# rqhuang88/DV-Matcher

Measured on AMD Instinct MI355X. Metric: point-cloud pairs/sec (N=2048, d=128), higher is better.
Workload: dtype f32; 1 GPU; BASELINE configs[1]: synthetic random pairs N=M=2048 d=128, correspondence+deform forward, both directions; deformer_weights=reference ckpt/dvmatcher_scape_r (fixture), fps_start=0, parallelism=pairs sharded over 1 GPU(s), no collective

## Files before the change

### dv-matcher_amd/csrc/dvm_grid.hip

```cpp
#include <stdlib.h>

#include <type_traits>

#include "dvm_common.h"

namespace dvm {

constexpr int GRID_T = 256;

template <class IndexT>
struct GridViewT {
    const float4 *pts;
    const IndexT *ids;
    const IndexT *start;
    float ox, oy, oz, h, scale2;
    int G;
};
typedef GridViewT<int32_t> GridView;
typedef GridViewT<uint16_t> GridViewLds;


static int grid_dim_for(int P) {
    int g = 2;
    while (g < 16 && (double)(g + 1) * (g + 1) * (g + 1) * 1.2 <= (double)P * 1.15) ++g;
    return g < 4 ? 4 : g;
}

struct GridBuildSets {
    const float *xyz[4];
    int Nsrc[4];
    GridBuf gb[4];
};
template <bool SETS>
__device__ __forceinline__ void grid_build_body(const float *__restrict__ xyz, int Nsrc, const int32_t *__restrict__ sel, const GridBuf &gb);
__global__ __launch_bounds__(GRID_T) void grid_build_sets_kernel(const GridBuildSets sets) {
    const int q = blockIdx.y;
    grid_build_body<true>(sets.xyz[q], sets.Nsrc[q], nullptr, sets.gb[q]);
}
__global__ __launch_bounds__(GRID_T) void grid_build_kernel(const float *__restrict__ xyz, int Nsrc,
                                                            const int32_t *__restrict__ sel, GridBuf gb) {
    grid_build_body<false>(xyz, Nsrc, sel, gb);
}
template <bool SETS>
__device__ __forceinline__ void grid_build_body(const float *__restrict__ xyz, int Nsrc, const int32_t *__restrict__ sel, const GridBuf &gb) {
    extern __shared__ int lds[];
    __shared__ float red[6][GRID_T / 64];
    __shared__ float par[8];
    __shared__ int wsum[GRID_T / 64];
    const int b = blockIdx.x, tid = threadIdx.x, lane = tid & 63, wave = tid >> 6;
    const int P = gb.P, G = gb.G, G3 = G * G * G;
    const float *p = xyz + (size_t)b * Nsrc * 3;
    const int32_t *sl = sel ? sel + (size_t)b * P : nullptr;
    constexpr int GC = 8;
    const bool cached = P <= GC * GRID_T;
    float px[GC], py[GC], pz[GC];
    if (cached) {
        int vs[GC];
#pragma unroll
        for (int q = 0; q < GC; ++q) {
            const int j = tid + q * GRID_T, jc = j < P ? j : P - 1;
            vs[q] = sl ? sl[jc] : jc;
        }
#pragma unroll
        for (int q = 0; q < GC; ++q) px[q] = p[3 * vs[q]], py[q] = p[3 * vs[q] + 1], pz[q] = p[3 * vs[q] + 2];
    }
    auto each_point = [&](auto &&f) __attribute__((always_inline)) {
        if (cached) {
#pragma unroll
            for (int q = 0; q < GC; ++q) {
                const int j = tid + q * GRID_T;
                if (j < P) f(j, px[q], py[q], pz[q]);
            }
        } else {
            for (int j = tid; j < P; j += GRID_T) {
                const int v = sl ? sl[j] : j;
                f(j, p[3 * v], p[3 * v + 1], p[3 * v + 2]);
            }
        }
    };
    float mn[3] = {INFINITY, INFINITY, INFINITY}, mx[3] = {-INFINITY, -INFINITY, -INFINITY};
    each_point([&](int, float x, float y, float z) {
        mn[0] = fminf(mn[0], x), mn[1] = fminf(mn[1], y), mn[2] = fminf(mn[2], z);
        mx[0] = fmaxf(mx[0], x), mx[1] = fmaxf(mx[1], y), mx[2] = fmaxf(mx[2], z);
    });
    for (int a = 0; a < 3; ++a) {
        for (int o = 32; o > 0; o >>= 1) {
            mn[a] = fminf(mn[a], __shfl_xor(mn[a], o, 64));
            mx[a] = fmaxf(mx[a], __shfl_xor(mx[a], o, 64));
        }
        if (lane == 0) {
            red[a][wave] = mn[a];
            red[3 + a][wave] = mx[a];
        }
    }
    __syncthreads();
    if (tid == 0) {
        float lo[3], hi[3];
        for (int a = 0; a < 3; ++a) {
            lo[a] = fminf(fminf(red[a][0], red[a][1]), fminf(red[a][2], red[a][3]));
            hi[a] = fmaxf(fmaxf(red[3 + a][0], red[3 + a][1]), fmaxf(red[3 + a][2], red[3 + a][3]));
        }
        float ext = fmaxf(fmaxf(hi[0] - lo[0], hi[1] - lo[1]), hi[2] - lo[2]);
        float h = ext > 0.f ? (ext / (float)G) * 1.000001f : 1.f;
        float m = 0.f;
        for (int a = 0; a < 3; ++a) m = fmaxf(m, fmaxf(fabsf(lo[a]), fabsf(hi[a])));
        par[0] = lo[0], par[1] = lo[1], par[2] = lo[2], par[3] = h, par[4] = 3.f * m * m + 1e-30f;
        for (int q = 0; q < 5; ++q) gb.params[(size_t)b * 8 + q] = par[q];
    }
    for (int c = tid; c <= G3; c += GRID_T) lds[c] = 0;
    __syncthreads();
    const float ox = par[0], oy = par[1], oz = par[2], inv = 1.0f / par[3];
    auto cell_of = [&](float x, float y, float z) {
        int cx = (int)((x - ox) * inv), cy = (int)((y - oy) * inv), cz = (int)((z - oz) * inv);
        cx = cx < 0 ? 0 : (cx > G - 1 ? G - 1 : cx);
        cy = cy < 0 ? 0 : (cy > G - 1 ? G - 1 : cy);
        cz = cz < 0 ? 0 : (cz > G - 1 ? G - 1 : cz);
        return (cz * G + cy) * G + cx;
    };
    each_point([&](int, float x, float y, float z) { atomicAdd(&lds[cell_of(x, y, z)], 1); });
    __syncthreads();
    const int chunk = (G3 + GRID_T - 1) / GRID_T;
    int local = 0;
    for (int c = tid * chunk; c < (tid + 1) * chunk && c < G3; ++c) local += lds[c];
    int inc = local;
    for (int o = 1; o < 64; o <<= 1) {
        int t = __shfl_up(inc, o, 64);
        if (lane >= o) inc += t;
    }
    if (lane == 63) wsum[wave] = inc;
    __syncthreads();
    int base = inc - local;
    for (int w2 = 0; w2 < wave; ++w2) base += wsum[w2];
    __syncthreads();
    int *cursor = lds + G3 + 1;
    int run = base;
    for (int c = tid * chunk; c < (tid + 1) * chunk && c < G3; ++c) {
        int cnt = lds[c];
        lds[c] = run;
        cursor[c] = run;
        run += cnt;
    }
    if (tid == 0) lds[G3] = P;
    __syncthreads();
    int32_t *st = gb.start + (size_t)b * (G3 + 1);
    for (int c = tid; c <= G3; c += GRID_T) st[c] = lds[c];
    float4 *op = gb.pts + (size_t)b * P;
    int32_t *oi = gb.ids + (size_t)b * P;
    each_point([&](int j, float x, float y, float z) {
        const int pos = atomicAdd(&cursor[cell_of(x, y, z)], 1);
        op[pos] = make_float4(x, y, z, sumsq3(x, y, z));
        oi[pos] = j;
    });
}

__device__ __forceinline__ GridView grid_view(const GridBuf &gb, int b) {
    GridView g;
    const int G3 = gb.G * gb.G * gb.G;
    g.pts = gb.pts + (size_t)b * gb.P;
    g.ids = gb.ids + (size_t)b * gb.P;
    g.start = gb.start + (size_t)b * (G3 + 1);
    const float *pr = gb.params + (size_t)b * 8;
    g.ox = pr[0], g.oy = pr[1], g.oz = pr[2], g.h = pr[3], g.scale2 = pr[4];
    g.G = gb.G;
    return g;
}

struct MetricMMQueryRow {
    typedef float key_t;
    float qx, qy, qz, nq;
    __device__ __forceinline__ void set(float x, float y, float z) { qx = x, qy = y, qz = z, nq = sumsq3(x, y, z); }
    __device__ __forceinline__ float operator()(const float4 &c) const {
        return sqrt_rn(d2_mm3(qx, qy, qz, nq, c.x, c.y, c.z, c.w));
    }
    __device__ __forceinline__ static float to_d2(float k) { return k * k; }
};
struct MetricMMCandRow {
    typedef float key_t;
    float qx, qy, qz, nq;
    __device__ __forceinline__ void set(float x, float y, float z) { qx = x, qy = y, qz = z, nq = sumsq3(x, y, z); }
    __device__ __forceinline__ float operator()(const float4 &c) const {
        return sqrt_rn(d2_mm3(c.x, c.y, c.z, c.w, qx, qy, qz, nq));
    }
    __device__ __forceinline__ static float to_d2(float k) { return k * k; }
};
struct MetricF64 {
    typedef double key_t;
    float qx, qy, qz;
    __device__ __forceinline__ void set(float x, float y, float z) { qx = x, qy = y, qz = z; }
    __device__ __forceinline__ double operator()(const float4 &c) const {
        double dx = (double)qx - (double)c.x, dy = (double)qy - (double)c.y, dz = (double)qz - (double)c.z;
        double s = 0.0;
        s = s + dx * dx;
        s = s + dy * dy;
        s = s + dz * dz;
        return s;
    }
    __device__ __forceinline__ static float to_d2(double k) { return (float)k; }
};
struct MetricF64Rounded {
    typedef float key_t;
    MetricF64 m;
    __device__ __forceinline__ void set(float x, float y, float z) { m.set(x, y, z); }
    __device__ __forceinline__ float operator()(const float4 &c) const { return (float)m(c); }
    __device__ __forceinline__ static float to_d2(float k) { return k; }
};
struct MetricDiff {
    typedef float key_t;
    float qx, qy, qz;
    __device__ __forceinline__ void set(float x, float y, float z) { qx = x, qy = y, qz = z; }
    __device__ __forceinline__ float operator()(const float4 &c) const { return d2_diff3(qx, qy, qz, c.x, c.y, c.z); }
    __device__ __forceinline__ static float to_d2(float k) { return k; }
};

template <class View, class Metric, class List>
__device__ __forceinline__ void grid_row(const View &g, const Metric &met, List &kb, int s0, int s1) {
    for (int s = s0; s < s1; ++s) kb.insert_lex(met(g.pts[s]), (int)g.ids[s]);
}

struct ChamferMin {
    float key;
    __device__ __forceinline__ float worst() const { return key; }
};
template <class Metric>
__device__ __forceinline__ void grid_row(const GridView &g, const Metric &met, ChamferMin &kb, int s0, int s1) {
    for (; s0 < s1; s0 += 4) {
        float4 pc[4];
#pragma unroll
        for (int u = 0; u < 4; ++u) pc[u] = g.pts[s0 + u < s1 ? s0 + u : s1 - 1];
#pragma unroll
        for (int u = 0; u < 4; ++u) kb.key = fminf(kb.key, s0 + u < s1 ? met(pc[u]) : INFINITY);
    }
}
struct ChamferMinPos {
    float key;
    int pos;
    __device__ __forceinline__ float worst() const { return key; }
};
template <class Metric>
__device__ __forceinline__ void grid_row(const GridView &g, const Metric &met, ChamferMinPos &kb, int s0, int s1) {
    for (int s = s0; s < s1; ++s) {
        const float v = met(g.pts[s]);
        if (v < kb.key) {
            kb.key = v, kb.pos = s;
        } else if (v == kb.key && (kb.pos < 0 || g.ids[s] < g.ids[kb.pos])) {
            kb.pos = s;
        }
    }
}

template <int K, class Metric, class List, class View>
__device__ __forceinline__ bool grid_search(const View &g, float qx, float qy, float qz, Metric &met, List &kb,
                                            int R0 = 1 , int Rmax = 1 << 30) {
    const int G = g.G;
    const float inv = 1.0f / g.h;
    int cx = (int)((qx - g.ox) * inv), cy = (int)((qy - g.oy) * inv), cz = (int)((qz - g.oz) * inv);
    cx = cx < 0 ? 0 : (cx > G - 1 ? G - 1 : cx);
    cy = cy < 0 ? 0 : (cy > G - 1 ? G - 1 : cy);
    cz = cz < 0 ? 0 : (cz > G - 1 ? G - 1 : cz);
    const float q2 = sumsq3(qx, qy, qz);
    const float margin = 64.f * 1.1920929e-7f * (g.scale2 + q2) + 1e-30f;
    int Rprev = R0 > 1 ? R0 - 1 : -1;
    for (int R = R0; R <= G && R <= Rmax; ++R) {
        const int x0 = cx - R < 0 ? 0 : cx - R, x1 = cx + R > G - 1 ? G - 1 : cx + R;
        const int y0 = cy - R < 0 ? 0 : cy - R, y1 = cy + R > G - 1 ? G - 1 : cy + R;
        const int z0 = cz - R < 0 ? 0 : cz - R, z1 = cz + R > G - 1 ? G - 1 : cz + R;
        for (int z = z0; z <= z1; ++z) {
            const float zlo = g.oz + (float)z * g.h;
            const float dz = fmaxf(0.f, fmaxf(zlo - qz, qz - (zlo + g.h)));
            for (int y = y0; y <= y1; ++y) {
                const float ylo = g.oy + (float)y * g.h;
                const float dy = fmaxf(0.f, fmaxf(ylo - qy, qy - (ylo + g.h)));
                if (Metric::to_d2(kb.worst()) < (dy * dy + dz * dz) * 0.9999f - margin) continue;
                const int rowbase = (z * G + y) * G;
                const bool inner_zy = (abs(z - cz) <= Rprev) && (abs(y - cy) <= Rprev);
                int sa0, sa1, sb0 = 0, sb1 = 0;
                if (inner_zy) {
                    const int ix0 = cx - Rprev < 0 ? 0 : cx - Rprev;
                    const int ix1 = cx + Rprev > G - 1 ? G - 1 : cx + Rprev;
                    sa0 = g.start[rowbase + x0];
                    sa1 = g.start[rowbase + ix0];
                    sb0 = g.start[rowbase + ix1 + 1];
                    sb1 = g.start[rowbase + x1 + 1];
                } else {
                    sa0 = g.start[rowbase + x0];
                    sa1 = g.start[rowbase + x1 + 1];
                }
                grid_row(g, met, kb, sa0, sa1);
                grid_row(g, met, kb, sb0, sb1);
            }
        }
        const float ext = (float)G * g.h;
        const float ex = fmaxf(0.f, fmaxf(g.ox - qx, qx - (g.ox + ext)));
        const float ey = fmaxf(0.f, fmaxf(g.oy - qy, qy - (g.oy + ext)));
        const float ez = fmaxf(0.f, fmaxf(g.oz - qz, qz - (g.oz + ext)));
        const float exx = ex * ex, eyy = ey * ey, ezz = ez * ez;
        float bound2 = INFINITY;
        auto face_x = [&](float f) { f = fmaxf(f, 0.f); bound2 = fminf(bound2, f * f + eyy + ezz); };
        auto face_y = [&](float f) { f = fmaxf(f, 0.f); bound2 = fminf(bound2, f * f + exx + ezz); };
        auto face_z = [&](float f) { f = fmaxf(f, 0.f); bound2 = fminf(bound2, f * f + exx + eyy); };
        if (cx - R >= 1) face_x(qx - (g.ox + (float)(cx - R) * g.h));
        if (cx + R < G - 1) face_x((g.ox + (float)(cx + R + 1) * g.h) - qx);
        if (cy - R >= 1) face_y(qy - (g.oy + (float)(cy - R) * g.h));
        if (cy + R < G - 1) face_y((g.oy + (float)(cy + R + 1) * g.h) - qy);
        if (cz - R >= 1) face_z(qz - (g.oz + (float)(cz - R) * g.h));
        if (cz + R < G - 1) face_z((g.oz + (float)(cz + R + 1) * g.h) - qz);
        if (bound2 == INFINITY) return true;
        const float kth = Metric::to_d2(kb.worst());
        if (kth < bound2 * 0.9999f - margin) return true;
        Rprev = R;
    }
    return Rmax >= G;
}

static __host__ __device__ __forceinline__ size_t grid_lds_bytes(int P, int G) {
    return ((size_t)P * (sizeof(float4) + sizeof(uint16_t)) + ((size_t)G * G * G + 1) * sizeof(uint16_t) + 15) / 16 * 16;
}
static size_t grid_lds_bytes(const GridBuf &gb) { return gb.P < 65536 ? grid_lds_bytes(gb.P, gb.G) : ~(size_t)0; }
__device__ __forceinline__ GridViewLds grid_stage_lds(const GridView &g, int P, char *lds, int threads) {
    const int G3 = g.G * g.G * g.G;
    float4 *lp = (float4 *)lds;
    uint16_t *li = (uint16_t *)(lds + (size_t)P * sizeof(float4));
    uint16_t *ls = li + P;
    for (int i = threadIdx.x; i < P; i += threads) lp[i] = g.pts[i], li[i] = (uint16_t)g.ids[i];
    for (int i = threadIdx.x; i <= G3; i += threads) ls[i] = (uint16_t)g.start[i];
    GridViewLds v;
    v.pts = lp, v.ids = li, v.start = ls;
    v.ox = g.ox, v.oy = g.oy, v.oz = g.oz, v.h = g.h, v.scale2 = g.scale2, v.G = g.G;
    return v;
}

template <int K, int THREADS = 128, bool LDS_GRID = false>
__global__ __launch_bounds__(THREADS) void grid_knn_self_kernel(GridBuf gb, int k, int32_t *__restrict__ idx) {
    extern __shared__ __attribute__((aligned(16))) char kn_lds[];
    const int b = blockIdx.y;
    const int t = blockIdx.x * blockDim.x + threadIdx.x;
    const int P = gb.P;
    const GridView gg = grid_view(gb, b);
    typename std::conditional<LDS_GRID, GridViewLds, GridView>::type g;
    if constexpr (LDS_GRID) {
        g = grid_stage_lds(gg, P, kn_lds, THREADS);
        __syncthreads();
    } else {
        g = gg;
    }
    if (t >= P) return;
    const float4 qp = g.pts[t];
    MetricMMQueryRow met;
    met.set(qp.x, qp.y, qp.z);
    KBestPacked<K> kb;
    kb.init(INFINITY);
    grid_search<K, MetricMMQueryRow>(g, qp.x, qp.y, qp.z, met, kb);
    int32_t *o = idx + ((size_t)b * P + g.ids[t]) * k;
    for (int q = 0; q < K; ++q)
        if (q < k) o[q] = (unsigned)kb.idx_at(q) < (unsigned)P ? kb.idx_at(q) : 0;
}

template <int THREADS = 128, bool LDS_GRID = false>
__global__ __launch_bounds__(THREADS) void grid_ring_kernel(GridBuf gb, int32_t *__restrict__ ring) {
    extern __shared__ __attribute__((aligned(16))) char rg_lds[];
    const int b = blockIdx.y;
    const int t = blockIdx.x * blockDim.x + threadIdx.x;
    const int P = gb.P;
    const GridView gg = grid_view(gb, b);
    typename std::conditional<LDS_GRID, GridViewLds, GridView>::type g;
    if constexpr (LDS_GRID) {
        g = grid_stage_lds(gg, P, rg_lds, THREADS);
        __syncthreads();
    } else {
        g = gg;
    }
    if (t >= P) return;
    const float4 qp = g.pts[t];
    const int a = g.ids[t];
    int32_t *o = ring + ((size_t)b * P + a) * 9;
    MetricF64Rounded mr;
    mr.set(qp.x, qp.y, qp.z);
    KBestPacked<10, 8> ks;
    ks.init(INFINITY);
    grid_search<9, MetricF64Rounded>(g, qp.x, qp.y, qp.z, mr, ks);
    bool ambiguous = false;
#pragma unroll
    for (int q = 0; q < 9; ++q) ambiguous = ambiguous || (ks.key_at(q) == ks.key_at(q + 1) && ks.key_at(q) < INFINITY);
    if (!ambiguous) {
        for (int q = 0; q < 9; ++q) o[q] = (unsigned)ks.idx_at(q) < (unsigned)P ? ks.idx_at(q) : a;
        return;
    }
    MetricF64 met;
    met.set(qp.x, qp.y, qp.z);
    KBest<9, double> kb;
    kb.init((double)INFINITY);
    grid_search<9, MetricF64>(g, qp.x, qp.y, qp.z, met, kb);
    for (int q = 0; q < 9; ++q) o[q] = (unsigned)kb.idx[q] < (unsigned)P ? kb.idx[q] : a;
}

template <int THREADS = 128, int LDS_GRID = 0>
__global__ __launch_bounds__(THREADS) void grid_infl_kernel(const float *__restrict__ xyz, int N, GridBuf gnodes, GridBuf gverts,
                                                            int32_t *__restrict__ infl, float *__restrict__ dists,
                                                            double *__restrict__ nnd) {
    extern __shared__ __attribute__((aligned(16))) char in_lds[];
    const int b = blockIdx.y;
    const int t = blockIdx.x * blockDim.x + threadIdx.x;
    const GridView gv0 = grid_view(gverts, b), gn0 = grid_view(gnodes, b);
    typename std::conditional<(LDS_GRID & 2) != 0, GridViewLds, GridView>::type gv;
    typename std::conditional<(LDS_GRID & 1) != 0, GridViewLds, GridView>::type gn;
    size_t used = 0;
    if constexpr ((LDS_GRID & 2) != 0) {
        gv = grid_stage_lds(gv0, gverts.P, in_lds, THREADS);
        used = grid_lds_bytes(gverts.P, gverts.G);
    } else {
        gv = gv0;
    }
    if constexpr ((LDS_GRID & 1) != 0) {
        gn = grid_stage_lds(gn0, gnodes.P, in_lds + used, THREADS);
    } else {
        gn = gn0;
    }
    if (LDS_GRID) __syncthreads();
    if (t >= N) return;
    const float4 qp = gv.pts[t];
    const int i = gv.ids[t];
    {
        MetricMMCandRow met;
        met.set(qp.x, qp.y, qp.z);
        KBestPacked<3> kb;
        kb.init(INFINITY);
        grid_search<3, MetricMMCandRow>(gn, qp.x, qp.y, qp.z, met, kb);
        const size_t row = (size_t)b * N + i;
        for (int q = 0; q < 3; ++q) {
            infl[row * 3 + q] = (unsigned)kb.idx_at(q) < (unsigned)gnodes.P ? kb.idx_at(q) : 0;
            dists[row * 3 + q] = kb.key_at(q);
        }
    }
    {
        MetricF64 met;
        met.set(qp.x, qp.y, qp.z);
        KBest<2, double> kb;
        kb.init((double)INFINITY);
        grid_search<2, MetricF64>(gv, qp.x, qp.y, qp.z, met, kb);
        nnd[(size_t)b * N + i] = sqrt(kb.key[1]);
    }
    (void)xyz;
}

struct ChGridGroup {
    GridBuf gq;
    GridBuf gb;
    float *dout;
    int32_t *iout;
};
struct ChGridArgs {
    ChGridGroup g[8];
    int scan_min;
    unsigned long long *stats;
};
typedef float f32x16_g __attribute__((ext_vector_type(16)));

template <bool WANT_IDX>
__device__ __forceinline__ void chamfer_exact_scan(const GridView &g, const MetricDiff &met, int s_begin, int s_end, float &best, int &bs) {
    for (int s0 = s_begin; s0 < s_end; s0 += 4) {
        float4 pc[4];
#pragma unroll
        for (int u = 0; u < 4; ++u) pc[u] = g.pts[s0 + u < s_end ? s0 + u : s_end - 1];
#pragma unroll
        for (int u = 0; u < 4; ++u) {
            const int sidx = s0 + u;
            const float d = sidx < s_end ? met(pc[u]) : INFINITY;
            if (!WANT_IDX) {
                best = fminf(best, d);
            } else if (d < best) {
                best = d, bs = sidx;
            } else if (d == best && d < INFINITY && g.ids[sidx] < g.ids[bs]) {
                bs = sidx;
            }
        }
    }
}

template <bool WANT_IDX>
__device__ __forceinline__ void chamfer_scan_wave(const ChGridGroup &G, const GridView &g, int b, int Na, bool done, const float4 qp, int i,
                                                  const MetricDiff &met, float margin, unsigned long long *stats, int grp) {
    const int P = G.gb.P;
    const int lane = threadIdx.x & 63, j32 = lane & 31, hh = lane >> 5;
    if (stats) {
        if (lane == 0) atomicAdd(stats + grp * 8 + 5, 1ull);
        if (!done) atomicAdd(stats + grp * 8 + 6, 1ull);
    }
    float bq[2][2];
#pragma unroll
    for (int tl = 0; tl < 2; ++tl) {
        const int src = j32 + 32 * tl;
        const float x = __shfl(qp.x, src, 64), y = __shfl(qp.y, src, 64), z = __shfl(qp.z, src, 64);
        bq[tl][0] = hh ? y : x;
        bq[tl][1] = hh ? 1.f : z;
    }
    float tb[2] = {INFINITY, INFINITY}, ts[2] = {INFINITY, INFINITY}, th[2] = {INFINITY, INFINITY};
    int tt[2] = {0, 0}, tu[2] = {0, 0};
    constexpr int TB = 4;
    float4 nx[TB];
#pragma unroll
    for (int u = 0; u < TB; ++u) {
        const int pi = 32 * u + j32;
        nx[u] = g.pts[pi < P ? pi : P - 1];
    }
    for (int s00 = 0; s00 < P; s00 += 32 * TB) {
        float4 cur[TB];
#pragma unroll
        for (int u = 0; u < TB; ++u) {
            cur[u] = nx[u];
            const int pi = s00 + 32 * (TB + u) + j32;
            nx[u] = g.pts[pi < P ? pi : P - 1];
        }
#pragma unroll
        for (int u = 0; u < TB; ++u) {
            const int s0 = s00 + 32 * u, pi = s0 + j32;
            const float4 pc = cur[u];
            const float pn = pi < P ? pc.w : INFINITY;
            const float a0 = hh ? -2.f * pc.y : -2.f * pc.x, a1 = hh ? pn : -2.f * pc.z;
#pragma unroll
            for (int tl = 0; tl < 2; ++tl) {
                f32x16_g acc = {0.f, 0.f, 0.f, 0.f, 0.f, 0.f, 0.f, 0.f, 0.f, 0.f, 0.f, 0.f, 0.f, 0.f, 0.f, 0.f};
                acc = __builtin_amdgcn_mfma_f32_32x32x2f32(a0, bq[tl][0], acc, 0, 0, 0);
                acc = __builtin_amdgcn_mfma_f32_32x32x2f32(a1, bq[tl][1], acc, 0, 0, 0);
                float m = fminf(fminf(fminf(acc[0], acc[1]), fminf(acc[2], acc[3])), fminf(fminf(acc[4], acc[5]), fminf(acc[6], acc[7])));
                m = fminf(m, fminf(fminf(fminf(acc[8], acc[9]), fminf(acc[10], acc[11])), fminf(fminf(acc[12], acc[13]), fminf(acc[14], acc[15]))));
                const bool lt1 = m < tb[tl], lt2 = m < ts[tl];
                th[tl] = lt2 ? ts[tl] : fminf(th[tl], m);
                tu[tl] = lt1 ? tt[tl] : (lt2 ? s0 : tu[tl]);
                ts[tl] = lt1 ? tb[tl] : (lt2 ? m : ts[tl]);
                tt[tl] = lt1 ? s0 : tt[tl];
                tb[tl] = lt1 ? m : tb[tl];
            }
        }
    }
    const float b1 = hh ? tb[1] : tb[0], s1 = hh ? ts[1] : ts[0], h1 = hh ? th[1] : th[0];
    const int t1 = hh ? tt[1] : tt[0], u1 = hh ? tu[1] : tu[0];
    const float b2 = __shfl_xor(hh ? tb[0] : tb[1], 32, 64), s2 = __shfl_xor(hh ? ts[0] : ts[1], 32, 64), h2 = __shfl_xor(hh ? th[0] : th[1], 32, 64);
    const int t2 = __shfl_xor(hh ? tt[0] : tt[1], 32, 64), u2 = __shfl_xor(hh ? tu[0] : tu[1], 32, 64);
    const float sbest = fminf(b1, b2);
    const int stile = b2 < b1 ? t2 : t1;
    const float c1 = t1 != stile ? b1 : INFINITY, c2 = u1 != stile ? s1 : INFINITY, c3 = t2 != stile ? b2 : INFINITY, c4 = u2 != stile ? s2 : INFINITY;
    const float ssec = fminf(fminf(c1, c2), fminf(c3, c4));
    const int stile2 = ssec == c1 ? t1 : (ssec == c2 ? u1 : (ssec == c3 ? t2 : u2));
    const float o1 = t1 != stile2 ? c1 : INFINITY, o2 = u1 != stile2 ? c2 : INFINITY, o3 = t2 != stile2 ? c3 : INFINITY, o4 = u2 != stile2 ? c4 : INFINITY;
    const float sother = fminf(fminf(h1, h2), fminf(fminf(o1, o2), fminf(o3, o4)));
    float best = INFINITY;
    int bs = 0;
    bool cert = false;
    if (!done) {
        chamfer_exact_scan<WANT_IDX>(g, met, stile, stile + 32 < P ? stile + 32 : P, best, bs);
        if (ssec < INFINITY) chamfer_exact_scan<WANT_IDX>(g, met, stile2, stile2 + 32 < P ? stile2 + 32 : P, best, bs);
        cert = sother - sbest > 2.f * margin;
    }
    if (__ballot(!done && !cert) != 0) {
        if (!done && !cert) {
            if (stats) atomicAdd(stats + grp * 8 + 7, 1ull);
            best = INFINITY, bs = 0;
            chamfer_exact_scan<WANT_IDX>(g, met, 0, P, best, bs);
        }
    }
    if (!done) {
        G.dout[(size_t)b * Na + i] = best;
        if (WANT_IDX && G.iout) G.iout[(size_t)b * Na + i] = g.ids[bs];
    }
}

template <int THREADS, bool LDS_TARGET, bool WANT_IDX>
__global__ __launch_bounds__(THREADS) void grid_chamfer_kernel(const ChGridArgs args) {
    extern __shared__ __attribute__((aligned(16))) char ch_lds[];
    const ChGridGroup &G = args.g[blockIdx.z];
    const int b = blockIdx.y;
    const int t = blockIdx.x * blockDim.x + threadIdx.x;
    const int Na = G.gq.P;
    const bool inrange = t < Na;
    GridView g = grid_view(G.gb, b);
    if (LDS_TARGET) {
        const int P = G.gb.P, G3 = G.gb.G * G.gb.G * G.gb.G;
        float4 *lp = (float4 *)ch_lds;
        int32_t *ls = (int32_t *)(ch_lds + (size_t)P * sizeof(float4));
        for (int i = threadIdx.x; i < P; i += THREADS) lp[i] = g.pts[i];
        for (int i = threadIdx.x; i <= G3; i += THREADS) ls[i] = g.start[i];
        __syncthreads();
        g.pts = lp;
        g.start = ls;
    }
    GridView q = grid_view(G.gq, b);
    const int tq = inrange ? t : Na - 1;
    const float4 qp = q.pts[tq];
    const int i = q.ids[tq];
    MetricDiff met;
    met.set(qp.x, qp.y, qp.z);
    const float q2 = sumsq3(qp.x, qp.y, qp.z);
    const float margin = 64.f * 1.1920929e-7f * (g.scale2 + q2) + 1e-30f;
    bool done = !inrange;
    float fbest = INFINITY;
    int fpos = -1;
    {
        const int Gd = g.G;
        const float inv = 1.0f / g.h;
        int cx = (int)((qp.x - g.ox) * inv), cy = (int)((qp.y - g.oy) * inv), cz = (int)((qp.z - g.oz) * inv);
        cx = cx < 0 ? 0 : (cx > Gd - 1 ? Gd - 1 : cx);
        cy = cy < 0 ? 0 : (cy > Gd - 1 ? Gd - 1 : cy);
        cz = cz < 0 ? 0 : (cz > Gd - 1 ? Gd - 1 : cz);
        const int x0 = cx - 1 < 0 ? 0 : cx - 1, x1 = cx + 1 > Gd - 1 ? Gd - 1 : cx + 1;
        int rs[9], re[9];
#pragma unroll
        for (int r = 0; r < 9; ++r) {
            const int z = cz + r / 3 - 1, y = cy + r % 3 - 1;
            const bool in = z >= 0 && z < Gd && y >= 0 && y < Gd;
            const int rowbase = ((in ? z : cz) * Gd + (in ? y : cy)) * Gd;
            rs[r] = g.start[rowbase + x0];
            const int rend = g.start[rowbase + x1 + 1];
            re[r] = in ? rend : rs[r];
        }
        float best = INFINITY;
        int bs = -1;
        bool tie = false;
        const float dlo[2] = {fmaxf(0.f, qp.y - (g.oy + (float)cy * g.h)), fmaxf(0.f, qp.z - (g.oz + (float)cz * g.h))};
        const float dhi[2] = {fmaxf(0.f, (g.oy + (float)(cy + 1) * g.h) - qp.y), fmaxf(0.f, (g.oz + (float)(cz + 1) * g.h) - qp.z)};
        constexpr int order[9] = {4, 1, 3, 5, 7, 0, 2, 6, 8};
        float rowb[9];
#pragma unroll
        for (int r = 0; r < 9; ++r) {
            const float dyr = r % 3 == 1 ? 0.f : (r % 3 == 0 ? dlo[0] : dhi[0]), dzr = r / 3 == 1 ? 0.f : (r / 3 == 0 ? dlo[1] : dhi[1]);
            rowb[r] = (dyr * dyr + dzr * dzr) * 0.9999f - margin;
        }
#pragma unroll
        for (int ri = 0; ri < 9; ++ri) {
            const int r = order[ri];
            if (best < rowb[r]) continue;
            const int rend = re[r];
            for (int s0 = rs[r]; s0 < rend; s0 += 4) {
                float4 pc[4];
#pragma unroll
                for (int u = 0; u < 4; ++u) pc[u] = g.pts[s0 + u < rend ? s0 + u : rend - 1];
#pragma unroll
                for (int u = 0; u < 4; ++u) {
                    const int s = s0 + u;
                    float dm = met(pc[u]);
                    asm volatile("" : "+v"(dm));
                    const bool inb = s < rend;
                    const float d = inb ? dm : INFINITY;
                    if (WANT_IDX) {
                        const bool lt = d < best, eq = d == best && inb && d < INFINITY;
                        tie = lt ? false : (tie || eq);
                        bs = lt ? s : bs;
                        best = lt ? d : best;
                    } else {
                        best = fminf(best, d);
                    }
                }
            }
        }
        if (WANT_IDX && tie && bs >= 0) {
            int bid = g.ids[bs];
#pragma unroll 1
            for (int r = 0; r < 9; ++r) {
                if (best < rowb[r]) continue;
                for (int s = rs[r]; s < re[r]; ++s) {
                    if (met(g.pts[s]) == best) {
                        const int id = g.ids[s];
                        if (id < bid) bid = id, bs = s;
                    }
                }
            }
        }
        const float ext = (float)Gd * g.h;
        const float ex = fmaxf(0.f, fmaxf(g.ox - qp.x, qp.x - (g.ox + ext)));
        const float ey = fmaxf(0.f, fmaxf(g.oy - qp.y, qp.y - (g.oy + ext)));
        const float ez = fmaxf(0.f, fmaxf(g.oz - qp.z, qp.z - (g.oz + ext)));
        const float exx = ex * ex, eyy = ey * ey, ezz = ez * ez;
        float bound2 = INFINITY;
        auto face = [&](float f, float o2) { f = fmaxf(f, 0.f); bound2 = fminf(bound2, f * f + o2); };
        if (cx - 1 >= 1) face(qp.x - (g.ox + (float)(cx - 1) * g.h), eyy + ezz);
        if (cx + 1 < Gd - 1) face((g.ox + (float)(cx + 2) * g.h) - qp.x, eyy + ezz);
        if (cy - 1 >= 1) face(qp.y - (g.oy + (float)(cy - 1) * g.h), exx + ezz);
        if (cy + 1 < Gd - 1) face((g.oy + (float)(cy + 2) * g.h) - qp.y, exx + ezz);
        if (cz - 1 >= 1) face(qp.z - (g.oz + (float)(cz - 1) * g.h), exx + eyy);
        if (cz + 1 < Gd - 1) face((g.oz + (float)(cz + 2) * g.h) - qp.z, exx + eyy);
        if (args.stats && inrange) {
            int ncand = 0;
#pragma unroll
            for (int r = 0; r < 9; ++r) ncand += re[r] - rs[r];
            atomicAdd(args.stats + blockIdx.z * 8 + 0, 1ull);
            atomicAdd(args.stats + blockIdx.z * 8 + 1, (unsigned long long)ncand);
        }
        const bool found = WANT_IDX ? bs >= 0 : best < INFINITY;
        if (found) fbest = best, fpos = bs;
        if (!done && found && (bound2 == INFINITY || best < bound2 * 0.9999f - margin)) {
            G.dout[(size_t)b * Na + i] = best;
            if (WANT_IDX && G.iout) G.iout[(size_t)b * Na + i] = g.ids[bs];
            done = true;
            if (args.stats) atomicAdd(args.stats + blockIdx.z * 8 + 2, 1ull);
        }
    }
    const int nfall = __popcll(__ballot(!done));
    if (nfall == 0) return;
    bool scan = nfall >= args.scan_min;
    if (!scan) {
        if (!done) {
            if (args.stats) atomicAdd(args.stats + blockIdx.z * 8 + 3, 1ull);
            typename std::conditional<WANT_IDX, ChamferMinPos, ChamferMin>::type kb;
            kb.key = fbest;
            if constexpr (WANT_IDX) kb.pos = fpos;
            if (grid_search<1, MetricDiff>(g, qp.x, qp.y, qp.z, met, kb, 2, 3)) {
                if (args.stats) atomicAdd(args.stats + blockIdx.z * 8 + 4, 1ull);
                G.dout[(size_t)b * Na + i] = kb.key;
                if constexpr (WANT_IDX)
                    if (G.iout) G.iout[(size_t)b * Na + i] = kb.pos >= 0 ? g.ids[kb.pos] : 0;
                done = true;
            }
        }
        scan = __ballot(!done) != 0;
        if (!scan) return;
    }
    chamfer_scan_wave<WANT_IDX>(G, g, b, Na, done, qp, i, met, margin, args.stats, blockIdx.z);
}

GridBuf grid_carve(Arena &ar, int B, int P) {
    GridBuf gb;
    gb.P = P;
    gb.G = grid_dim_for(P);
    const int G3 = gb.G * gb.G * gb.G;
    gb.pts = ar.take<float4>((size_t)B * P);
    gb.ids = ar.take<int32_t>((size_t)B * P);
    gb.start = ar.take<int32_t>((size_t)B * (G3 + 1));
    gb.params = ar.take<float>((size_t)B * 8);
    return gb;
}
size_t grid_bytes(int B, int P) {
    Arena ar(nullptr, 0);
    grid_carve(ar, B, P);
    return ar.off;
}

void launch_grid_build_sets(const float *const *xyz, const int *Nsrc, const GridBuf *gb, int nsets, int B, hipStream_t s) {
    GridBuildSets sets;
    size_t lds = 0;
    for (int q = 0; q < 4; ++q) {
        const int r = q < nsets ? q : 0;
        sets.xyz[q] = xyz[r], sets.Nsrc[q] = Nsrc[r], sets.gb[q] = gb[r];
        const int G3 = gb[r].G * gb[r].G * gb[r].G;
        const size_t nb = (size_t)(2 * G3 + 1) * sizeof(int);
        lds = nb > lds ? nb : lds;
    }
    hipLaunchKernelGGL(grid_build_sets_kernel, dim3(B, nsets), dim3(GRID_T), lds, s, sets);
}
void launch_grid_build(const float *xyz, int B, int Nsrc, const int32_t *sel, const GridBuf &gb, hipStream_t s) {
    const int G3 = gb.G * gb.G * gb.G;
    size_t lds = (size_t)(2 * G3 + 1) * sizeof(int);
    hipLaunchKernelGGL(grid_build_kernel, dim3(B), dim3(GRID_T), lds, s, xyz, Nsrc, sel, gb);
}

template <int K>
static void launch_knn_self_k(const GridBuf &gb, int B, int k, int32_t *idx, hipStream_t s) {
    const size_t lds = grid_lds_bytes(gb);
    if (lds <= 64 * 1024) {
        ensure_dyn_lds((const void *)grid_knn_self_kernel<K, 512, true>, (int)lds);
        hipLaunchKernelGGL((grid_knn_self_kernel<K, 512, true>), dim3((gb.P + 511) / 512, B), dim3(512), lds, s, gb, k, idx);
    } else {
        hipLaunchKernelGGL((grid_knn_self_kernel<K, 128, false>), dim3((gb.P + 127) / 128, B), dim3(128), 0, s, gb, k, idx);
    }
}

void launch_grid_knn_self(const GridBuf &gb, int B, int k, int32_t *idx, hipStream_t s) {
    prof_begin(s, DVM_PROF_KNN_XYZ);
    if (k <= 3)
        launch_knn_self_k<3>(gb, B, k, idx, s);
    else if (k <= 10)
        launch_knn_self_k<10>(gb, B, k, idx, s);
    else
        launch_knn_self_k<16>(gb, B, k, idx, s);
    prof_end(s, DVM_PROF_KNN_XYZ);
}

void launch_grid_ring(const GridBuf &gnodes, int B, int32_t *ring, hipStream_t s) {
    const size_t lds = grid_lds_bytes(gnodes);
    if (lds <= 64 * 1024) {
        ensure_dyn_lds((const void *)grid_ring_kernel<512, true>, (int)lds);
        hipLaunchKernelGGL((grid_ring_kernel<512, true>), dim3((gnodes.P + 511) / 512, B), dim3(512), lds, s, gnodes, ring);
    } else {
        hipLaunchKernelGGL((grid_ring_kernel<128, false>), dim3((gnodes.P + 127) / 128, B), dim3(128), 0, s, gnodes, ring);
    }
}

void launch_grid_infl(const float *xyz, int B, int N, const GridBuf &gnodes, const GridBuf &gverts, int32_t *infl, float *dists,
                      double *nnd, hipStream_t s) {
    const size_t lds = grid_lds_bytes(gnodes);
    if (lds <= 64 * 1024) {
        ensure_dyn_lds((const void *)grid_infl_kernel<512, 1>, (int)lds);
        hipLaunchKernelGGL((grid_infl_kernel<512, 1>), dim3((N + 511) / 512, B), dim3(512), lds, s, xyz, N, gnodes, gverts, infl, dists, nnd);
    } else {
        hipLaunchKernelGGL((grid_infl_kernel<128, 0>), dim3((N + 127) / 128, B), dim3(128), 0, s, xyz, N, gnodes, gverts, infl, dists, nnd);
    }
}

void launch_grid_chamfer(const GridBuf *gq, const GridBuf *gb, float *const *dout, int32_t *const *iout, int ngroups, int B,
                         hipStream_t s) {
    ChGridArgs args;
    int maxN = 1;
    for (int q = 0; q < 8; ++q) {
        int r = q < ngroups ? q : 0;
        args.g[q] = ChGridGroup{gq[r], gb[r], dout[r], iout ? iout[r] : nullptr};
        if (q < ngroups && gq[r].P > maxN) maxN = gq[r].P;
    }
    bool want_idx = false;
    for (int q = 0; q < ngroups; ++q) want_idx = want_idx || args.g[q].iout != nullptr;
    args.scan_min = 24;
    args.stats = nullptr;
    if ((options().debug & DVM_DEBUG_CHAMFER_STATS) && hipMalloc(&args.stats, 64 * sizeof(unsigned long long)) == hipSuccess)
        (void)hipMemsetAsync(args.stats, 0, 64 * sizeof(unsigned long long), s);
    size_t lds_bytes = 0;
    for (int q = 0; q < ngroups; ++q) {
        const size_t nb = (size_t)gb[q].P * sizeof(float4) + ((size_t)gb[q].G * gb[q].G * gb[q].G + 1) * sizeof(int32_t);
        lds_bytes = nb > lds_bytes ? nb : lds_bytes;
    }
    lds_bytes = (lds_bytes + 15) / 16 * 16;
    prof_begin(s, DVM_PROF_CHAMFER);
    const dim3 grid_lds((maxN + 511) / 512, B, ngroups), grid_glb((maxN + 127) / 128, B, ngroups);
    if (lds_bytes <= 64 * 1024 && want_idx) {
        ensure_dyn_lds((const void *)grid_chamfer_kernel<512, true, true>, (int)lds_bytes);
        hipLaunchKernelGGL((grid_chamfer_kernel<512, true, true>), grid_lds, dim3(512), lds_bytes, s, args);
    } else if (lds_bytes <= 64 * 1024) {
        ensure_dyn_lds((const void *)grid_chamfer_kernel<512, true, false>, (int)lds_bytes);
        hipLaunchKernelGGL((grid_chamfer_kernel<512, true, false>), grid_lds, dim3(512), lds_bytes, s, args);
    } else if (want_idx) {
        hipLaunchKernelGGL((grid_chamfer_kernel<128, false, true>), grid_glb, dim3(128), 0, s, args);
    } else {
        hipLaunchKernelGGL((grid_chamfer_kernel<128, false, false>), grid_glb, dim3(128), 0, s, args);
    }
    prof_end(s, DVM_PROF_CHAMFER);
    if (args.stats) {
        unsigned long long h[64];
        (void)hipStreamSynchronize(s);
        (void)hipMemcpy(h, args.stats, sizeof(h), hipMemcpyDeviceToHost);
        for (int q = 0; q < ngroups; ++q)
            fprintf(stderr, "chamfer group %d: %llu queries, %.1f radius-1 candidates each, %.1f%% certified there, %.1f%% walked (%.1f%% certified by the walk), "
                            "%llu waves scanned for %llu lanes, %llu exact fallbacks\n", q, h[q * 8], (double)h[q * 8 + 1] / (double)(h[q * 8] ? h[q * 8] : 1),
                    100.0 * h[q * 8 + 2] / (h[q * 8] ? h[q * 8] : 1), 100.0 * h[q * 8 + 3] / (h[q * 8] ? h[q * 8] : 1),
                    100.0 * h[q * 8 + 4] / (h[q * 8] ? h[q * 8] : 1), h[q * 8 + 5], h[q * 8 + 6], h[q * 8 + 7]);
        (void)hipFree(args.stats);
    }
}

}
```

Measured before the change: 56880 pairs/s.

## Search on squared distances and float rank with exact fallback for ties

The kNN-self and influence-node searches now rank candidates by squared distance, avoiding a correctly-rounded sqrt per candidate. They keep one extra slot, take the roots only for the final list, re-sort it, and fall back to the original rooted search only for lanes with ties at the boundary. The second-nearest-vertex search ranks with a float-rounded f64 metric using packed lists and recomputes exact doubles for the top three, running the full f64 search only when ties are detected. This adds extra list width, a fixup sort and divergent fallback paths, and bit-exactness depends on the tie detection being complete.

```diff
diff --git a/dv-matcher_amd/csrc/dvm_grid.hip b/dv-matcher_amd/csrc/dvm_grid.hip
--- a/dv-matcher_amd/csrc/dvm_grid.hip
+++ b/dv-matcher_amd/csrc/dvm_grid.hip
@@ -165,24 +165,32 @@
     return g;
 }
 
-struct MetricMMQueryRow {
+template <bool ROOT>
+struct MetricMMQueryRowT {
     typedef float key_t;
     float qx, qy, qz, nq;
     __device__ __forceinline__ void set(float x, float y, float z) { qx = x, qy = y, qz = z, nq = sumsq3(x, y, z); }
     __device__ __forceinline__ float operator()(const float4 &c) const {
-        return sqrt_rn(d2_mm3(qx, qy, qz, nq, c.x, c.y, c.z, c.w));
-    }
-    __device__ __forceinline__ static float to_d2(float k) { return k * k; }
-};
-struct MetricMMCandRow {
+        const float d2 = d2_mm3(qx, qy, qz, nq, c.x, c.y, c.z, c.w);
+        return ROOT ? sqrt_rn(d2) : d2;
+    }
+    __device__ __forceinline__ static float to_d2(float k) { return ROOT ? k * k : k; }
+};
+template <bool ROOT>
+struct MetricMMCandRowT {
     typedef float key_t;
     float qx, qy, qz, nq;
     __device__ __forceinline__ void set(float x, float y, float z) { qx = x, qy = y, qz = z, nq = sumsq3(x, y, z); }
     __device__ __forceinline__ float operator()(const float4 &c) const {
-        return sqrt_rn(d2_mm3(c.x, c.y, c.z, c.w, qx, qy, qz, nq));
-    }
-    __device__ __forceinline__ static float to_d2(float k) { return k * k; }
-};
+        const float d2 = d2_mm3(c.x, c.y, c.z, c.w, qx, qy, qz, nq);
+        return ROOT ? sqrt_rn(d2) : d2;
+    }
+    __device__ __forceinline__ static float to_d2(float k) { return ROOT ? k * k : k; }
+};
+typedef MetricMMQueryRowT<true> MetricMMQueryRow;
+typedef MetricMMQueryRowT<false> MetricMMQueryRowSq;
+typedef MetricMMCandRowT<true> MetricMMCandRow;
+typedef MetricMMCandRowT<false> MetricMMCandRowSq;
 struct MetricF64 {
     typedef double key_t;
     float qx, qy, qz;
@@ -215,6 +223,13 @@
 template <class View, class Metric, class List>
 __device__ __forceinline__ void grid_row(const View &g, const Metric &met, List &kb, int s0, int s1) {
     for (int s = s0; s < s1; ++s) kb.insert_lex(met(g.pts[s]), (int)g.ids[s]);
+}
+
+template <int K, int W>
+struct KBestPackedPos : KBestPacked<K, W> {};
+template <class View, class Metric, int K, int W>
+__device__ __forceinline__ void grid_row(const View &g, const Metric &met, KBestPackedPos<K, W> &kb, int s0, int s1) {
+    for (int s = s0; s < s1; ++s) kb.insert_lex(met(g.pts[s]), s);
 }
 
 struct ChamferMin {
@@ -329,6 +344,42 @@
     return v;
 }
 
+template <int K1>
+__device__ __forceinline__ bool finish_squared_keys(KBestPacked<K1, K1 - 2> &kb, int k) {
+    typedef KBestPacked<K1, K1 - 2> L;
+#pragma unroll
+    for (int q = 0; q < K1; ++q) kb.e[q] = __hiloint2double(__float_as_int(sqrt_rn(kb.key_at(q))) + L::KBIAS, kb.idx_at(q));
+    bool ambiguous = false, inverted = false;
+#pragma unroll
+    for (int q = 0; q + 1 < K1; ++q) {
+        ambiguous = ambiguous || (q == k - 1 && kb.key_at(q) == kb.key_at(q + 1) && kb.key_at(q) < INFINITY);
+        inverted = inverted || kb.e[q + 1] < kb.e[q];
+    }
+    if (__ballot(inverted) != 0) {
+#pragma unroll 1
+        for (int it = 0; it < (K1 + 1) / 2; ++it) {
+#pragma unroll
+            for (int par = 0; par < 2; ++par)
+#pragma unroll
+                for (int p = par; p + 1 < K1; p += 2) {
+                    const double lo = L::mn(kb.e[p], kb.e[p + 1]), hi = L::mx(kb.e[p], kb.e[p + 1]);
+                    kb.e[p] = lo, kb.e[p + 1] = hi;
+                }
+        }
+    }
+    return ambiguous;
+}
+
+template <int K, class View>
+__device__ __forceinline__ void knn_self_rooted(const View &g, const float4 qp, int k, int P, int32_t *__restrict__ o) {
+    MetricMMQueryRow met;
+    met.set(qp.x, qp.y, qp.z);
+    KBestPacked<K> kb;
+    kb.init(INFINITY);
+    grid_search<K, MetricMMQueryRow>(g, qp.x, qp.y, qp.z, met, kb);
+    for (int q = 0; q < K; ++q)
+        if (q < k) o[q] = (unsigned)kb.idx_at(q) < (unsigned)P ? kb.idx_at(q) : 0;
+}
 template <int K, int THREADS = 128, bool LDS_GRID = false>
 __global__ __launch_bounds__(THREADS) void grid_knn_self_kernel(GridBuf gb, int k, int32_t *__restrict__ idx) {
     extern __shared__ __attribute__((aligned(16))) char kn_lds[];
@@ -345,14 +396,19 @@
     }
     if (t >= P) return;
     const float4 qp = g.pts[t];
-    MetricMMQueryRow met;
+    int32_t *o = idx + ((size_t)b * P + g.ids[t]) * k;
+    MetricMMQueryRowSq met;
     met.set(qp.x, qp.y, qp.z);
-    KBestPacked<K> kb;
+    KBestPacked<K + 1, K - 1> kb;
     kb.init(INFINITY);
-    grid_search<K, MetricMMQueryRow>(g, qp.x, qp.y, qp.z, met, kb);
-    int32_t *o = idx + ((size_t)b * P + g.ids[t]) * k;
-    for (int q = 0; q < K; ++q)
-        if (q < k) o[q] = (unsigned)kb.idx_at(q) < (unsigned)P ? kb.idx_at(q) : 0;
+    grid_search<K, MetricMMQueryRowSq>(g, qp.x, qp.y, qp.z, met, kb);
+    const bool ambiguous = finish_squared_keys(kb, k);
+    if (!ambiguous)
+        for (int q = 0; q < K; ++q)
+            if (q < k) o[q] = (unsigned)kb.idx_at(q) < (unsigned)P ? kb.idx_at(q) : 0;
+    if (__ballot(ambiguous) != 0) {
+        if (ambiguous) knn_self_rooted<K>(g, qp, k, P, o);
+    }
 }
 
 template <int THREADS = 128, bool LDS_GRID = false>
@@ -393,6 +449,18 @@
     for (int q = 0; q < 9; ++q) o[q] = (unsigned)kb.idx[q] < (unsigned)P ? kb.idx[q] : a;
 }
 
+template <class View>
+__device__ __forceinline__ void infl_rooted(const View &gn, const float4 qp, int Pn, int32_t *__restrict__ infl, float *__restrict__ dists) {
+    MetricMMCandRow met;
+    met.set(qp.x, qp.y, qp.z);
+    KBestPacked<3> kb;
+    kb.init(INFINITY);
+    grid_search<3, MetricMMCandRow>(gn, qp.x, qp.y, qp.z, met, kb);
+    for (int q = 0; q < 3; ++q) {
+        infl[q] = (unsigned)kb.idx_at(q) < (unsigned)Pn ? kb.idx_at(q) : 0;
+        dists[q] = kb.key_at(q);
+    }
+}
 template <int THREADS = 128, int LDS_GRID = 0>
 __global__ __launch_bounds__(THREADS) void grid_infl_kernel(const float *__restrict__ xyz, int N, GridBuf gnodes, GridBuf gverts,
                                                             int32_t *__restrict__ infl, float *__restrict__ dists,
@@ -420,24 +488,50 @@
     const float4 qp = gv.pts[t];
     const int i = gv.ids[t];
     {
-        MetricMMCandRow met;
+        const size_t row = (size_t)b * N + i;
+        MetricMMCandRowSq met;
         met.set(qp.x, qp.y, qp.z);
-        KBestPacked<3> kb;
+        KBestPacked<4, 2> kb;
         kb.init(INFINITY);
-        grid_search<3, MetricMMCandRow>(gn, qp.x, qp.y, qp.z, met, kb);
-        const size_t row = (size_t)b * N + i;
-        for (int q = 0; q < 3; ++q) {
-            infl[row * 3 + q] = (unsigned)kb.idx_at(q) < (unsigned)gnodes.P ? kb.idx_at(q) : 0;
-            dists[row * 3 + q] = kb.key_at(q);
+        grid_search<3, MetricMMCandRowSq>(gn, qp.x, qp.y, qp.z, met, kb);
+        const bool ambiguous = finish_squared_keys(kb, 3);
+        if (!ambiguous)
+            for (int q = 0; q < 3; ++q) {
+                infl[row * 3 + q] = (unsigned)kb.idx_at(q) < (unsigned)gnodes.P ? kb.idx_at(q) : 0;
+                dists[row * 3 + q] = kb.key_at(q);
+            }
+        if (__ballot(ambiguous) != 0) {
+            if (ambiguous) infl_rooted(gn, qp, gnodes.P, infl + row * 3, dists + row * 3);
         }
     }
     {
         MetricF64 met;
         met.set(qp.x, qp.y, qp.z);
-        KBest<2, double> kb;
-        kb.init((double)INFINITY);
-        grid_search<2, MetricF64>(gv, qp.x, qp.y, qp.z, met, kb);
-        nnd[(size_t)b * N + i] = sqrt(kb.key[1]);
+        MetricF64Rounded mr;
+        mr.set(qp.x, qp.y, qp.z);
+        KBestPackedPos<4, 1> ks;
+        ks.init(INFINITY);
+        grid_search<2, MetricF64Rounded>(gv, qp.x, qp.y, qp.z, mr, ks);
+        const bool ambiguous = ks.key_at(3) == ks.key_at(1) && ks.key_at(1) < INFINITY;
+        double m1 = (double)INFINITY, m2 = (double)INFINITY;
+#pragma unroll
+        for (int q = 0; q < 3; ++q) {
+            const int s = ks.idx_at(q);
+            const bool has = (unsigned)s < (unsigned)N;
+            const double v = met(gv.pts[has ? s : 0]);
+            const double vv = has && v == v ? v : (double)INFINITY;
+            m2 = vv < m1 ? m1 : (vv < m2 ? vv : m2);
+            m1 = vv < m1 ? vv : m1;
+        }
+        if (!ambiguous) nnd[(size_t)b * N + i] = sqrt(m2);
+        if (__ballot(ambiguous) != 0) {
+            if (ambiguous) {
+                KBest<2, double> kb;
+                kb.init((double)INFINITY);
+                grid_search<2, MetricF64>(gv, qp.x, qp.y, qp.z, met, kb);
+                nnd[(size_t)b * N + i] = sqrt(kb.key[1]);
+            }
+        }
     }
     (void)xyz;
 }
```

Measured after the change: 56810 pairs/s, median of 2. Within noise of the previous version (-0.1%).

## Use split-f16 MFMA for chamfer tile screening with scaled certification margin

Applied to the files above, without the earlier changes.

Replaces the two f32 32x32x2 MFMAs per tile in the chamfer screening sweep with a single 32x32x16 f16 MFMA. Coordinates are scaled by a power of two and split into high and low f16 parts, so each tile gets an approximate squared-distance bound. The certification margin is widened to cover the f16 rounding error, and the f32 path stays as a fallback when the scale is not finite. It also swaps the min reduction and top-3 tracking for inline min3/med3 asm and changes the prefetch to a double-buffered TB=2 sweep. The risk is more exact-rescan fallbacks if the widened margin fails certification more often.

```diff
diff --git a/dv-matcher_amd/csrc/dvm_grid.hip b/dv-matcher_amd/csrc/dvm_grid.hip
--- a/dv-matcher_amd/csrc/dvm_grid.hip
+++ b/dv-matcher_amd/csrc/dvm_grid.hip
@@ -3,6 +3,7 @@
 #include <type_traits>
 
 #include "dvm_common.h"
+#include "dvm_mlp_f16.h"
 
 namespace dvm {
 
@@ -454,6 +455,8 @@
     unsigned long long *stats;
 };
 typedef float f32x16_g __attribute__((ext_vector_type(16)));
+typedef _Float16 f16x8_g __attribute__((ext_vector_type(8)));
+typedef unsigned u32x4_g __attribute__((ext_vector_type(4)));
 
 template <bool WANT_IDX>
 __device__ __forceinline__ void chamfer_exact_scan(const GridView &g, const MetricDiff &met, int s_begin, int s_end, float &best, int &bs) {
@@ -476,6 +479,33 @@
     }
 }
 
+__device__ __forceinline__ float fmin2i(float a, float b) {
+    float r;
+    asm("v_min_f32 %0, %1, %2" : "=v"(r) : "v"(a), "v"(b));
+    return r;
+}
+__device__ __forceinline__ float acc_min16(const f32x16_g &acc, float inf) {
+    const float last = __builtin_canonicalizef(acc[15]);
+    float r0, r1, r2;
+    asm("v_min3_f32 %0, %3, %4, %5\n\t"
+        "v_min3_f32 %1, %6, %7, %8\n\t"
+        "v_min3_f32 %2, %9, %10, %11\n\t"
+        "v_min3_f32 %0, %0, %1, %2\n\t"
+        "v_min3_f32 %1, %12, %13, %14\n\t"
+        "v_min3_f32 %2, %15, %16, %17\n\t"
+        "v_min3_f32 %1, %1, %2, %18\n\t"
+        "v_min3_f32 %0, %0, %1, %19"
+        : "=&v"(r0), "=&v"(r1), "=&v"(r2)
+        : "v"(acc[0]), "v"(acc[1]), "v"(acc[2]), "v"(acc[3]), "v"(acc[4]), "v"(acc[5]), "v"(acc[6]), "v"(acc[7]), "v"(acc[8]),
+          "v"(acc[9]), "v"(acc[10]), "v"(acc[11]), "v"(acc[12]), "v"(acc[13]), "v"(acc[14]), "v"(last), "v"(inf));
+    return r0;
+}
+__device__ __forceinline__ float fmed3i(float a, float b, float c) {
+    float r;
+    asm("v_med3_f32 %0, %1, %2, %3" : "=v"(r) : "v"(a), "v"(b), "v"(c));
+    return r;
+}
+
 template <bool WANT_IDX>
 __device__ __forceinline__ void chamfer_scan_wave(const ChGridGroup &G, const GridView &g, int b, int Na, bool done, const float4 qp, int i,
                                                   const MetricDiff &met, float margin, unsigned long long *stats, int grp) {
@@ -485,52 +515,94 @@
         if (lane == 0) atomicAdd(stats + grp * 8 + 5, 1ull);
         if (!done) atomicAdd(stats + grp * 8 + 6, 1ull);
     }
-    float bq[2][2];
-#pragma unroll
-    for (int tl = 0; tl < 2; ++tl) {
-        const int src = j32 + 32 * tl;
-        const float x = __shfl(qp.x, src, 64), y = __shfl(qp.y, src, 64), z = __shfl(qp.z, src, 64);
-        bq[tl][0] = hh ? y : x;
-        bq[tl][1] = hh ? 1.f : z;
-    }
     float tb[2] = {INFINITY, INFINITY}, ts[2] = {INFINITY, INFINITY}, th[2] = {INFINITY, INFINITY};
     int tt[2] = {0, 0}, tu[2] = {0, 0};
-    constexpr int TB = 4;
-    float4 nx[TB];
-#pragma unroll
-    for (int u = 0; u < TB; ++u) {
-        const int pi = 32 * u + j32;
-        nx[u] = g.pts[pi < P ? pi : P - 1];
-    }
-    for (int s00 = 0; s00 < P; s00 += 32 * TB) {
-        float4 cur[TB];
+    const float finf = INFINITY;
+    auto keep = [&](int tl, float m, int s0) {
+        const bool lt1 = m < tb[tl], lt2 = m < ts[tl];
+        int tun = lt2 ? s0 : tu[tl];
+        asm volatile("" : "+v"(tun));
+        tu[tl] = lt1 ? tt[tl] : tun;
+        tt[tl] = lt1 ? s0 : tt[tl];
+        th[tl] = fmed3i(ts[tl], th[tl], m);
+        ts[tl] = fmed3i(tb[tl], ts[tl], m);
+        tb[tl] = fmin2i(tb[tl], m);
+    };
+    constexpr int TB = 2;
+    auto fetch = [&](float4 (&buf)[TB], int s00) {
 #pragma unroll
         for (int u = 0; u < TB; ++u) {
-            cur[u] = nx[u];
-            const int pi = s00 + 32 * (TB + u) + j32;
-            nx[u] = g.pts[pi < P ? pi : P - 1];
-        }
-#pragma unroll
-        for (int u = 0; u < TB; ++u) {
-            const int s0 = s00 + 32 * u, pi = s0 + j32;
-            const float4 pc = cur[u];
-            const float pn = pi < P ? pc.w : INFINITY;
-            const float a0 = hh ? -2.f * pc.y : -2.f * pc.x, a1 = hh ? pn : -2.f * pc.z;
+            const int pi = s00 + j32, last = P - 1 - 32 * u;
+            buf[u] = g.pts[(pi < last ? pi : last) + 32 * u];
+        }
+    };
+    auto sweep = [&](auto &&unit) {
+        float4 pa[TB], pb[TB];
+        fetch(pa, 0);
+        for (int s00 = 0; s00 < P; s00 += 64 * TB) {
+            fetch(pb, s00 + 32 * TB);
+#pragma unroll
+            for (int u = 0; u < TB; ++u) {
+                if (s00 + 32 * u >= P) break;
+                unit(pa[u], s00 + 32 * u);
+            }
+            fetch(pa, s00 + 64 * TB);
+#pragma unroll
+            for (int u = 0; u < TB; ++u) {
+                if (s00 + 32 * (TB + u) >= P) break;
+                unit(pb[u], s00 + 32 * (TB + u));
+            }
+        }
+    };
+    float q2m = sumsq3(qp.x, qp.y, qp.z);
+#pragma unroll
+    for (int o = 32; o > 0; o >>= 1) q2m = fmaxf(q2m, __shfl_xor(q2m, o, 64));
+    const int r2bits = __builtin_amdgcn_readfirstlane(__float_as_int(fmaxf(g.scale2, q2m)));
+    const bool f16 = r2bits < 0x7f800000;
+    const int ks = (25 - ((r2bits >> 23) - 127)) >> 1;
+    const float sc2 = f16 ? __int_as_float((2 * ks + 127) << 23) : 1.f;
+    if (f16) {
+        const float sq = __int_as_float((ks + 127) << 23), sx = -2.f * sq, sn = __int_as_float((2 * ks - 12 + 127) << 23);
+        f16x8_g bq[2];
+#pragma unroll
+        for (int tl = 0; tl < 2; ++tl) {
+            const int src = j32 + 32 * tl;
+            const float x = __shfl(qp.x, src, 64), y = __shfl(qp.y, src, 64), z = __shfl(qp.z, src, 64);
+            unsigned h01, m01, h23, m23;
+            split2x2(sq * x, sq * y, h01, m01);
+            split2x2(sq * z, 4096.f, h23, m23);
+            bq[tl] = __builtin_bit_cast(f16x8_g, u32x4_g{hh ? 0u : h01, hh ? 0u : h23, hh ? m01 : h01, hh ? m23 : h23});
+        }
+        sweep([&](const float4 &pc, int s0) {
+            unsigned h01, m01, h23, m23;
+            split2x2(sx * pc.x, sx * pc.y, h01, m01);
+            split2x2(sx * pc.z, sn * pc.w, h23, m23);
+            const f16x8_g a = __builtin_bit_cast(f16x8_g, u32x4_g{hh ? 0u : h01, hh ? 0u : h23, hh ? h01 : m01, hh ? h23 : m23});
+            const f32x16_g zero = {0.f, 0.f, 0.f, 0.f, 0.f, 0.f, 0.f, 0.f, 0.f, 0.f, 0.f, 0.f, 0.f, 0.f, 0.f, 0.f};
+            const f32x16_g acc0 = __builtin_amdgcn_mfma_f32_32x32x16_f16(a, bq[0], zero, 0, 0, 0);
+            const f32x16_g acc1 = __builtin_amdgcn_mfma_f32_32x32x16_f16(a, bq[1], zero, 0, 0, 0);
+            keep(0, acc_min16(acc0, finf), s0);
+            keep(1, acc_min16(acc1, finf), s0);
+        });
+    } else {
+        float bq[2][2];
+#pragma unroll
+        for (int tl = 0; tl < 2; ++tl) {
+            const int src = j32 + 32 * tl;
+            const float x = __shfl(qp.x, src, 64), y = __shfl(qp.y, src, 64), z = __shfl(qp.z, src, 64);
+            bq[tl][0] = hh ? -2.f * y : -2.f * x;
+            bq[tl][1] = hh ? 1.f : -2.f * z;
+        }
+        sweep([&](const float4 &pc, int s0) {
+            const float a0 = hh ? pc.y : pc.x, a1 = hh ? pc.w : pc.z;
 #pragma unroll
             for (int tl = 0; tl < 2; ++tl) {
                 f32x16_g acc = {0.f, 0.f, 0.f, 0.f, 0.f, 0.f, 0.f, 0.f, 0.f, 0.f, 0.f, 0.f, 0.f, 0.f, 0.f, 0.f};
                 acc = __builtin_amdgcn_mfma_f32_32x32x2f32(a0, bq[tl][0], acc, 0, 0, 0);
                 acc = __builtin_amdgcn_mfma_f32_32x32x2f32(a1, bq[tl][1], acc, 0, 0, 0);
-                float m = fminf(fminf(fminf(acc[0], acc[1]), fminf(acc[2], acc[3])), fminf(fminf(acc[4], acc[5]), fminf(acc[6], acc[7])));
-                m = fminf(m, fminf(fminf(fminf(acc[8], acc[9]), fminf(acc[10], acc[11])), fminf(fminf(acc[12], acc[13]), fminf(acc[14], acc[15]))));
-                const bool lt1 = m < tb[tl], lt2 = m < ts[tl];
-                th[tl] = lt2 ? ts[tl] : fminf(th[tl], m);
-                tu[tl] = lt1 ? tt[tl] : (lt2 ? s0 : tu[tl]);
-                ts[tl] = lt1 ? tb[tl] : (lt2 ? m : ts[tl]);
-                tt[tl] = lt1 ? s0 : tt[tl];
-                tb[tl] = lt1 ? m : tb[tl];
+                keep(tl, acc_min16(acc, finf), s0);
             }
-        }
+        });
     }
     const float b1 = hh ? tb[1] : tb[0], s1 = hh ? ts[1] : ts[0], h1 = hh ? th[1] : th[0];
     const int t1 = hh ? tt[1] : tt[0], u1 = hh ? tu[1] : tu[0];
@@ -549,7 +621,7 @@
     if (!done) {
         chamfer_exact_scan<WANT_IDX>(g, met, stile, stile + 32 < P ? stile + 32 : P, best, bs);
         if (ssec < INFINITY) chamfer_exact_scan<WANT_IDX>(g, met, stile2, stile2 + 32 < P ? stile2 + 32 : P, best, bs);
-        cert = sother - sbest > 2.f * margin;
+        cert = sother - sbest > 2.f * (f16 ? margin * sc2 + 4.f : margin);
     }
     if (__ballot(!done && !cert) != 0) {
         if (!done && !cert) {
```

Result: faster. 56800 pairs/s before, 58270 pairs/s after, median of 6 (+2.6%).
